# fskovbo/OptimalControlMPS

Measured on NVIDIA B200. Metric: cost+gradient evals/s (BH N=20 chi=100), higher is better.
Workload: dtype complex128 (f64)

## Files before the change

optimalcontrolmps_b200/csrc/decomp.cu:

```cuda
#include <cstdio>
#include <cstdlib>
#include "ocmps_internal.h"

__device__ unsigned long long g_jac_dbg[8];
__device__ double g_jac_flops[2];

namespace {

constexpr int JAC_THREADS = 512;
constexpr int JAC_EPL = 8;
constexpr int JAC_NV_SMEM = 512;
constexpr int JAC_MAX_SWEEPS = 60;
constexpr int JAC_BLOCKED_ROWS = 64;
constexpr double JAC_TOL2 = 1e-28;
constexpr double DEFLATE_REL = 1e-30;
constexpr int NV_MAX = 2048;
constexpr int BJ_C = 8;
constexpr int BJ_TPP = 4;
constexpr int BJ_MAX_ROWS = 256;
constexpr int BJ_SLOTS = BJ_MAX_ROWS / 2;
constexpr int BJ_THREADS = BJ_SLOTS * BJ_TPP;
constexpr int BJ_MAX_EPL = 8;
constexpr int BJ_MIN_CAP = 112;

__host__ __device__ __forceinline__ int gc_ldy(int len) { int l = (len + 3) & ~3; if ((l & 7) == 0) l += 4; return l; }
__host__ __device__ __forceinline__ int gc_ldg(int nvp) { return nvp | 1; }
__device__ __forceinline__ void gc_dmma(double& d0, double& d1, double a, double b) {
  asm volatile("mma.sync.aligned.m8n8k4.row.col.f64.f64.f64.f64 {%0,%1}, {%2}, {%3}, {%0,%1};\n" : "+d"(d0), "+d"(d1) : "d"(a), "d"(b));
// ... 249 lines not shown
      rb[e].x = __shfl_xor_sync(0xffffffffu, rb[e].x, 16);
      rb[e].y = __shfl_xor_sync(0xffffffffu, rb[e].y, 16);
    }
    nbn = __shfl_xor_sync(0xffffffffu, nbn, 16);
    rowB = __shfl_xor_sync(0xffffffffu, rowB, 16);
    jac_rotate<EPL>(ra, rb, na, nbn, rowA >= 0 && rowB >= 0, thr, hl, s_rot, s_big);
    int NP = -1, NQ = -1;
    if (R + 1 < nbp - 1) {
      blocks_of(R + 1, NP, NQ);
      if ((NP >= 0 && NP == hbB) || (NQ >= 0 && NQ == hbA)) { const int t = NP; NP = NQ; NQ = t; }
    }
    if (hbA != NP) store_row(ra, na, rowA);
    if (hbB != NQ) store_row(rb, nbn, rowB);
    P = NP; Q = NQ;
    __syncthreads();
  }
}

struct QrState {
  cplx* Y;
  int nv, len;
  double rtol_abs;
  double *ncur, *nnext, *nrmref, *rdr, *rdi;
  short *perm, *pcur, *pnext;
  unsigned long long (*s_cand)[32];
};

template <int EPL, int E0>
__device__ __forceinline__ bool qr_step_cached(const QrState& q, int j) {
  constexpr unsigned long long KEY_POS = 2047ull;
  constexpr int nwarps = JAC_THREADS / 32;
  const int tid = threadIdx.x, lane = tid & 31, warp = tid >> 5, half = lane >> 4, hl = lane & 15;
  const int len = q.len, nv = q.nv;
  int bpos;
  {
    const unsigned long long kk = q.s_cand[j & 1][lane];
    const unsigned khi = (unsigned)(kk >> 32);
    const unsigned mhi = __reduce_max_sync(0xffffffffu, khi);
    const unsigned mlo = __reduce_max_sync(0xffffffffu, khi == mhi ? (unsigned)kk : 0u);
    bpos = (int)(KEY_POS - (unsigned long long)(mlo & 2047u));
  }
  const int pv = q.pcur[bpos];
  const int pj = q.pcur[j];
  const cplx* x = q.Y + pv * len;
  const cplx alpha = x[j];
  cplx xv[EPL];
  double sq0 = 0.0, sq1 = 0.0;
#pragma unroll
  for (int e = E0; e < EPL; ++e) {
    const int c = hl + 16 * e;
    const bool in = (e > E0 || c >= j) && (e < EPL - 1 || c < len);
    xv[e] = x[in ? c : j];
    if (!in) xv[e] = make_double2(0.0, 0.0);
    const double q2 = xv[e].x * xv[e].x + xv[e].y * xv[e].y;
    if ((e - E0) & 1) sq1 += q2; else sq0 += q2;
  }
  const double best = half_sum(sq0 + sq1);
  if (!(best > q.rtol_abs)) return false;
  const double inx = rsqrt(best), normx = best * inx;
  const double a2 = alpha.x * alpha.x + alpha.y * alpha.y;
  const double ia = a2 > 0.0 ? rsqrt(a2) : 0.0, aabs = a2 * ia;
  const double phr = a2 > 0.0 ? alpha.x * ia : 1.0, phi = a2 > 0.0 ? alpha.y * ia : 0.0;
  const double dr = phr * normx, di = phi * normx;
  const double v0r = alpha.x + dr, v0i = alpha.y + di;
  const double rb = rsqrt(normx * (normx + aabs));
  const double beta = rb * rb;
  if (tid == 0) { q.rdr[j] = -dr; q.rdi[j] = -di; q.perm[j] = (short)pv; }
  unsigned long long cand = 0ull;
  for (int ib = j + 1 + 2 * warp; ib < nv; ib += 2 * nwarps) {
    const int i = ib + half;
    const bool act = i < nv;
    const int phys = act ? (i == bpos ? pj : (int)q.pcur[i]) : pv;
    cplx* y = q.Y + phys * len;
    const cplx yj = y[j];
    const double told = q.ncur[phys], tref = q.nrmref[phys];
    cplx yv[EPL];
    double w0r = 0.0, w0i = 0.0, w1r = 0.0, w1i = 0.0;
#pragma unroll
    for (int e = E0; e < EPL; ++e) {
      const int c = hl + 16 * e;
      if (e < EPL - 1) yv[e] = y[c];
      else { yv[e] = y[c < len ? c : j]; if (c >= len) yv[e] = make_double2(0.0, 0.0); }
      const double pr = xv[e].x * yv[e].x + xv[e].y * yv[e].y;
      const double pi = xv[e].x * yv[e].y - xv[e].y * yv[e].x;
      if ((e - E0) & 1) { w1r += pr; w1i += pi; } else { w0r += pr; w0i += pi; }
    }
    double wr = half_sum(w0r + w1r), wi = half_sum(w0i + w1i);
    wr += dr * yj.x + di * yj.y;
    wi += dr * yj.y - di * yj.x;
    const double fr = beta * wr, fi = beta * wi;
// ... 144 lines not shown
  }
  __syncthreads();
  if (tid == 0) {
    double t = 0.0;
    for (int v = 0; v < nv; ++v) t += nrm[v];
    s_F = t;
    s_keff = 0;
  }
  __syncthreads();
  const double F = s_F;
  const double rtol_abs = F * rank_tol;

  const long long t_qr0 = clock64();
  const int kmax = nv < len ? nv : len;
  int keff = 0;
  double* ncur = nrm;  double* nnext = nrm2;
  short* pcur = permA; short* pnext = permB;
  constexpr unsigned long long KEY_POS = 2047ull;
  const bool qr_cached = CACHED && len <= 16 * JAC_EPL;
  if (qr_cached) {
    QrState q;
    q.Y = Y; q.nv = nv; q.len = len; q.rtol_abs = rtol_abs;
    q.ncur = ncur; q.nnext = nnext; q.nrmref = nrmref; q.rdr = rdr; q.rdi = rdi;
    q.perm = perm; q.pcur = pcur; q.pnext = pnext; q.s_cand = s_cand;
    switch ((len + 15) >> 4) {
      case 1: keff = qr_pivoted_cached<1>(q); break;
      case 2: keff = qr_pivoted_cached<2>(q); break;
      case 3: keff = qr_pivoted_cached<3>(q); break;
      case 4: keff = qr_pivoted_cached<4>(q); break;
      case 5: keff = qr_pivoted_cached<5>(q); break;
      case 6: keff = qr_pivoted_cached<6>(q); break;
      case 7: keff = qr_pivoted_cached<7>(q); break;
      default: keff = qr_pivoted_cached<8>(q); break;
    }
    ncur = q.ncur; nnext = q.nnext; pcur = q.pcur; pnext = q.pnext;
  }
  if (tid < 3) s_key[tid] = 0ull;
  __syncthreads();
  for (int v = tid; v < nv; v += JAC_THREADS)
    atomicMax(&s_key[0], ((unsigned long long)__double_as_longlong(nrm[v]) & ~KEY_POS) | (KEY_POS - (unsigned long long)v));
  __syncthreads();
  for (int j = 0; j < (qr_cached ? 0 : kmax); ++j) {
    const int bpos = (int)(KEY_POS - (s_key[j % 3] & KEY_POS));
    if (tid == 0) s_key[(j + 2) % 3] = 0ull;
    const int pv = pcur[bpos];
    const int pj = pcur[j];
// ... 49 lines not shown
      if (act) {
        tnew = ncur[phys] - rji2;
        redo = !(tnew > 1.5e-8 * nrmref[phys]);
      }
      if (__any_sync(0xffffffffu, redo)) {
        double tail = 0.0;
        if (act && redo) for (int c = j + 1 + hl; c < len; c += 16) { const cplx yy = y[c]; tail += yy.x * yy.x + yy.y * yy.y; }
        tail = half_sum(tail);
        if (act && redo) { tnew = tail; if (hl == 0) nrmref[phys] = tail; }
      }
      if (act && hl == 0) {
        tnew = tnew > 0.0 ? tnew : 0.0;
        nnext[phys] = tnew; pnext[i] = (short)phys;
        atomicMax(knext, ((unsigned long long)__double_as_longlong(tnew) & ~KEY_POS) | (KEY_POS - (unsigned long long)i));
      }
    }
    }
    __syncthreads();
    { double* t = ncur; ncur = nnext; nnext = t; short* u = pcur; pcur = pnext; pnext = u; }
  }
  for (int i = keff + tid; i < nv; i += JAC_THREADS) perm[i] = pcur[i];
  __syncthreads();
  if (tid == 0) s_keff = keff;

  const int ldz = CACHED ? ldpad : nv;
  for (int e = tid; e < keff * ldz; e += JAC_THREADS) {
    const int c = e / ldz, i = e % ldz;
    cplx v = make_double2(0.0, 0.0);
    if (i == c) v = make_double2(rdr[c], rdi[c]);
    else if (i > c && i < nv) v = Y[(int)perm[i] * len + c];
    Yb[e] = v;
  }
  __syncthreads();
  {
    double* hF = b.scratch_d + 7 * NV_MAX;
    int* hK = reinterpret_cast<int*>(b.scratch_d + 7 * NV_MAX + OCMPS_MAX_BLK);
    int* hB = hK + OCMPS_MAX_BLK;
    int* hS = hB + OCMPS_MAX_BLK;
    const bool handover_small = CACHED && keff <= JAC_BLOCKED_ROWS;
    const bool handover_big = !handover_small && big_on && keff <= BJ_MAX_ROWS && nv <= BJ_MAX_ROWS;
    const bool handover = handover_small || handover_big;
    if (tid == 0) {
      hF[blockIdx.x] = F;
      hK[blockIdx.x] = handover_small ? keff : -1;
      hB[blockIdx.x] = handover_big ? keff : -1;
      hS[blockIdx.x] = ldz;
// ... 1219 lines not shown
  extern __shared__ __align__(16) unsigned char smem_raw[];
  __shared__ RcShared sh;
  const int blk = (int)blockIdx.x / RC_C;
  const unsigned rank = clus::cluster_rank();
  const int keff = rot_handover_rows(b, blk, smem_elems);
  if (keff < 0) return;
  if (keff < RC_MIN_ROWS) {
    if (rank == 0) jacobi_rot_block(a, b, blk, keff, smem_raw);
    return;
  }
  cplx* Zs = reinterpret_cast<cplx*>(smem_raw);
  switch ((b.dw->blk[blk].nv + 15) >> 4) {
    case 1: rc_run<1>(a, b, blk, keff, rank, Zs, sh); break;
    case 2: rc_run<2>(a, b, blk, keff, rank, Zs, sh); break;
    case 3: rc_run<3>(a, b, blk, keff, rank, Zs, sh); break;
    case 4: rc_run<4>(a, b, blk, keff, rank, Zs, sh); break;
    case 5: rc_run<5>(a, b, blk, keff, rank, Zs, sh); break;
    case 6: rc_run<6>(a, b, blk, keff, rank, Zs, sh); break;
    case 7: rc_run<7>(a, b, blk, keff, rank, Zs, sh); break;
    default: rc_run<8>(a, b, blk, keff, rank, Zs, sh); break;
  }
}

__global__ void __launch_bounds__(1024) truncate_kernel(DecompArgs a, DecompBuffers b, TruncParams tp) {
  __shared__ double cP[NV_MAX];
  __shared__ double sSorted[NV_MAX];
  __shared__ short cQ[NV_MAX], cI[NV_MAX], cI2[NV_MAX];
  __shared__ unsigned char sKeep[NV_MAX];
  __shared__ int sBlkOff[OCMPS_MAX_BLK + 1];
  __shared__ double sWarp[32];
  __shared__ int sWarpCnt[33];
  __shared__ double s_docut, s_kept;
  __shared__ int s_nfinal;
  DecompWork* w = b.dw;
  const int nv = w->nvtot;
  const int nblocks = w->nblocks;
  const int tid = threadIdx.x, lane = tid & 31, warp = tid >> 5;
  for (int i = tid; i < nblocks; i += blockDim.x) sBlkOff[i] = w->blk[i].p_off;
  if (tid == 0) { s_nfinal = 0; s_docut = 0.0; }
  const int i0 = 2 * tid, i1 = i0 + 1;
  const double p0 = i0 < nv ? b.P[i0] : 0.0, p1 = i1 < nv ? b.P[i1] : 0.0;
  const int f0 = p0 > 0.0, f1 = p1 > 0.0;
  int incl = f0 + f1;
#pragma unroll
  for (int o = 1; o < 32; o <<= 1) { const int up = __shfl_up_sync(0xffffffffu, incl, o); if (lane >= o) incl += up; }
  if (lane == 31) sWarpCnt[warp + 1] = incl;
// ... 152 lines not shown
      for (int i = 0; i < 32; ++i) t += sWarp[i];
      s_kept = t;
    }
    __syncthreads();
  }
  if (tid == 0) {
    int k = total;
    if (k == 0 && nv > 0) {
      k = 1;
      a.qNew[0] = b.vecq[0];
      inv_blk[0] = 0;
      inv_v[0] = 0;
    }
    if (k > tp.cap) { atomicOr(b.status, OCMPS_ST_CAPACITY); k = tp.cap; }
    w->newdim = k;
    *a.dimNew = k;
    const double kept = s_kept;
    double scale = 1.0;
    if (tp.normalize) {
      const double nrm = sqrt(kept);
      if (nrm > 1e-16) scale = 1.0 / nrm;
    }
    w->scale = scale;
    const int n = w->n, m = w->m;
    GemmDesc g1;
    g1.pad = 0;
    g1.A = g1.B = nullptr; g1.C = nullptr; g1.M = g1.N = g1.K = 0; g1.lda = g1.ldb = g1.ldc = 1; g1.opA = g1.opB = 0;
    if (a.kind == DK_ORTH_LEFT) {
      const int far = a.D * (*a.dimNb);
      g1.A = a.partner; g1.opA = 0; g1.lda = m;
      g1.B = a.nb_in; g1.opB = 0; g1.ldb = far;
      g1.C = a.nb_out; g1.ldc = far; g1.M = k; g1.N = far; g1.K = m;
    } else if (a.kind == DK_ORTH_RIGHT) {
      const int far = a.D * (*a.dimNb);
      g1.A = a.nb_in; g1.opA = 0; g1.lda = n;
      g1.B = a.partner; g1.opB = 0; g1.ldb = k;
      g1.C = a.nb_out; g1.ldc = k; g1.M = far; g1.N = k; g1.K = n;
    }
    b.descs[1] = g1;
  }
}

constexpr int BUILD_THREADS = 512;
__global__ void __launch_bounds__(BUILD_THREADS) build_factors_kernel(DecompArgs a, DecompBuffers b) {
  extern __shared__ __align__(16) unsigned char bsm[];
  __shared__ double red[BUILD_THREADS / 32];
  __shared__ double s_inv;
  const DecompWork* w = b.dw;
  const int k = w->newdim;
  const int kk = blockIdx.x;
  if (kk >= k) return;
  const int n = w->n, m = w->m, ld = w->ld, mode = w->mode;
  const int* comp_blk = b.comp_idx + NV_MAX;
  const int* comp_rank = b.comp_idx + 2 * NV_MAX;
  const int* vec_blk = b.vec_idx + NV_MAX;
  const int* vec_rank = b.vec_idx + 2 * NV_MAX;
  const int bi = b.pos[NV_MAX + kk], j = b.pos[2 * NV_MAX + kk];
  const DecompBlock B = w->blk[bi];
  const int nv = B.nv, len = B.len;
  const cplx* Zj = b.ywork + B.ws_off + (size_t)j * nv;
  const double sigma = sqrt(b.P[B.p_off + j]) * w->scale;
  cplx* zs = reinterpret_cast<cplx*>(bsm);
  cplx* out = zs + nv;
  int* vidx = reinterpret_cast<int*>(out + len);
  int* cidx = vidx + nv;
  const int tid = threadIdx.x, lane = tid & 31, wp = tid >> 5;
  constexpr int NW = BUILD_THREADS / 32;
  for (int v = tid; v < nv; v += BUILD_THREADS) { zs[v] = Zj[v]; vidx[v] = b.vec_idx[B.vec_off + v]; }
  for (int c = tid; c < len; c += BUILD_THREADS) cidx[c] = b.comp_idx[B.comp_off + c];
  __syncthreads();
  double part = 0.0;
  if (mode == 0) {
    for (int c = wp; c < len; c += NW) {
      const cplx* row = a.X + (size_t)cidx[c] * ld;
      double sr = 0.0, si = 0.0;
      for (int v0 = 0; v0 < nv; v0 += 128) {
        cplx x[4];
#pragma unroll
        for (int u = 0; u < 4; ++u) {
          const int v = v0 + lane + 32 * u;
          x[u] = make_double2(0.0, 0.0);
          if (v < nv) x[u] = row[vidx[v]];
        }
#pragma unroll
        for (int u = 0; u < 4; ++u) {
          const int v = v0 + lane + 32 * u;
          if (v < nv) {
            const cplx z = zs[v];
            sr += x[u].x * z.x + x[u].y * z.y;
            si += x[u].y * z.x - x[u].x * z.y;
          }
        }
      }
      sr = warp_sum(sr); si = warp_sum(si);
      if (lane == 0) { out[c] = make_double2(sr, si); part += sr * sr + si * si; }
// ... 4 lines not shown
      const int c = c0 + cl;
      const bool in = c < len;
      const cplx* colp = a.X + (in ? cidx[c] : 0);
      double sr = 0.0, si = 0.0;
      if (in) {
#pragma unroll 4
        for (int v = g; v < nv; v += 4) {
          const cplx x = colp[(size_t)vidx[v] * ld], z = zs[v];
          sr += x.x * z.x + x.y * z.y;
          si += x.y * z.x - x.x * z.y;
        }
      }
      sr += __shfl_xor_sync(0xffffffffu, sr, 8);  si += __shfl_xor_sync(0xffffffffu, si, 8);
      sr += __shfl_xor_sync(0xffffffffu, sr, 16); si += __shfl_xor_sync(0xffffffffu, si, 16);
      if (in && g == 0) { out[c] = make_double2(sr, si); part += sr * sr + si * si; }
    }
  }
  part = warp_sum(part);
  if ((tid & 31) == 0) red[tid >> 5] = part;
  __syncthreads();
  if (tid == 0) {
    double t = 0.0;
    for (int i = 0; i < BUILD_THREADS / 32; ++i) t += red[i];
    s_inv = t > 0.0 ? rsqrt(t) : 0.0;
  }
  __syncthreads();
  const double inv = s_inv;
  const int ncomp = mode == 0 ? n : m, nvec = mode == 0 ? m : n;
  for (int c = tid; c < ncomp; c += BUILD_THREADS) {
    cplx v = make_double2(0.0, 0.0);
    if (comp_blk[c] == bi) { const cplx o = out[comp_rank[c]]; v = make_double2(o.x * inv, o.y * inv); }
    if (mode == 0) a.iso[(size_t)c * k + kk] = v; else a.iso[(size_t)kk * m + c] = v;
  }
  if (a.qNb != nullptr && (a.kind == DK_ORTH_LEFT || a.kind == DK_ORTH_RIGHT)) {
    const int D = a.D, chiFar = *a.dimNb, qj = B.q;
    if (a.kind == DK_ORTH_LEFT) {
      const long long far = (long long)D * chiFar;
      for (int r = tid; r < chiFar; r += BUILD_THREADS) {
        const int sx = a.qNb[r] - qj;
        double ar = 0.0, ai = 0.0;
        if (sx >= 0 && sx < D) {
          const cplx* col = a.nb_in + (long long)sx * chiFar + r;
#pragma unroll 4
          for (int t = 0; t < nv; ++t) {
            const cplx z = zs[t], x = col[(long long)vidx[t] * far];
            ar += z.x * x.x - z.y * x.y;
            ai += z.x * x.y + z.y * x.x;
// ... 70 lines not shown
}

int grid_for(long long elems, int threads, int cap = 1184) {
  long long g = (elems + threads - 1) / threads;
  if (g < 1) g = 1;
  if (g > cap) g = cap;
  return (int)g;
}

}

static bool g_jac_attr_set[64] = {false};

void debug_jacobi_counters(unsigned long long* out, bool reset) {
  cudaMemcpyFromSymbol(out, g_jac_dbg, sizeof(unsigned long long) * 8);
  if (reset) { unsigned long long z[8] = {0}; cudaMemcpyToSymbol(g_jac_dbg, z, sizeof(z)); }
}

void debug_row_cluster_counters(unsigned long long* out, bool reset) {
  cudaMemcpyFromSymbol(out, g_rc_dbg, sizeof(unsigned long long) * 2);
  if (reset) { unsigned long long z[2] = {0, 0}; cudaMemcpyToSymbol(g_rc_dbg, z, sizeof(z)); }
}

__global__ void __launch_bounds__(256) spectrum_entropy_kernel(DecompBuffers b, double* out) {
  __shared__ double red[256];
  const int nv = b.dw->nvtot;
  double acc = 0.0;
  for (int i = threadIdx.x; i < nv; i += 256) {
    const double p = b.P[i];
    if (p > 1e-12) acc -= p * log(p);
  }
  red[threadIdx.x] = acc;
  __syncthreads();
  for (int o = 128; o > 0; o >>= 1) {
    if ((int)threadIdx.x < o) red[threadIdx.x] += red[threadIdx.x + o];
    __syncthreads();
  }
  if (threadIdx.x == 0) *out = red[0];
}

void launch_spectrum_entropy(const DecompBuffers& b, double* out, cudaStream_t s) {
  spectrum_entropy_kernel<<<1, 256, 0, s>>>(b, out);
}

void launch_decomp_setup(const DecompArgs& a, const DecompBuffers& b, cudaStream_t s) {
  decomp_setup_kernel<<<1, SETUP_THREADS, 0, s>>>(a, b);
// ... 38 lines not shown
    }
    e0 = g_prof_events[g_prof_used].first; e1 = g_prof_events[g_prof_used].second;
    ++g_prof_used;
    cudaEventRecord(e0, s);
  }
  struct Tail { cudaEvent_t e; cudaStream_t s; ~Tail() { if (e) cudaEventRecord(e, s); } } tail{e1, s};
  int dev = 0;
  cudaGetDevice(&dev);
  static std::mutex attr_mu;
  if (dev < 64) {
  std::lock_guard<std::mutex> attr_lock(attr_mu);
  if (!g_jac_attr_set[dev]) {
    cudaFuncSetAttribute(jacobi_blocks_kernel<true, true>, cudaFuncAttributeMaxDynamicSharedMemorySize, 200 * 1024);
    cudaFuncSetAttribute(jacobi_blocks_kernel<true, false>, cudaFuncAttributeMaxDynamicSharedMemorySize, 200 * 1024);
    cudaFuncSetAttribute(build_factors_kernel, cudaFuncAttributeMaxDynamicSharedMemorySize, 96 * 1024);
    cudaFuncSetAttribute(jacobi_rot_kernel, cudaFuncAttributeMaxDynamicSharedMemorySize, (int)(JAC_BLOCKED_ROWS * 16 * JAC_EPL * sizeof(cplx)));
    cudaFuncSetAttribute(jacobi_rows_cluster_kernel, cudaFuncAttributeMaxDynamicSharedMemorySize, (int)(JAC_BLOCKED_ROWS * 16 * JAC_EPL * sizeof(cplx)));
    cudaFuncSetAttribute(jacobi_big_kernel, cudaFuncAttributeMaxDynamicSharedMemorySize, (int)(BJ_MAX_ROWS * (BJ_TPP * BJ_MAX_EPL + 4) * sizeof(cplx)));
    cudaFuncSetAttribute(qr_big_kernel, cudaFuncAttributeMaxDynamicSharedMemorySize, (int)((32 * BJ_MAX_ROWS + BJ_MAX_ROWS) * sizeof(cplx)));
    g_jac_attr_set[dev] = true;
  }
  }
  static const bool big_env = [] { const char* e = getenv("OCMPS_BIG_CLUSTER"); return !(e && e[0] == '0'); }();
  int big_on = (big_env && max_rows >= BJ_MIN_CAP) ? 1 : 0;
  static const bool gram_env = [] { const char* e = getenv("OCMPS_GRAM"); return e && e[0] == '1'; }();
  if (gram_env && (a.kind == DK_GATE_LEFT || a.kind == DK_GATE_RIGHT)) big_on |= 2;
  static const bool fork_env = [] { const char* e = getenv("OCMPS_SVD_FORK"); return !(e && e[0] == '0'); }();
  const bool forked = fork_env && (big_on & 1) && fork && fork->stream;
  cudaStream_t sb = forked ? fork->stream : s;
  if (forked) { cudaEventRecord(fork->ev_fork, s); cudaStreamWaitEvent(sb, fork->ev_fork, 0); }
  jacobi_blocks_kernel<true, true><<<nblk_launch, JAC_THREADS, smem_limit, s>>>(a, b, (int)(smem_limit / sizeof(cplx)), rank_tol, big_on);
  if (forked) cudaEventRecord(fork->ev_first, s);
  if (long_rows) jacobi_blocks_kernel<true, false><<<nblk_launch, JAC_THREADS, smem_limit, s>>>(a, b, (int)(smem_limit / sizeof(cplx)), rank_tol, big_on);
  if (need_global) jacobi_blocks_kernel<false, false><<<nblk_launch, JAC_THREADS, 0, s>>>(a, b, (int)(smem_limit / sizeof(cplx)), rank_tol, big_on);
  if (big_on & 1) {
    cudaLaunchConfig_t cfg = {};
    cfg.gridDim = dim3(nblk_launch * BJ_C, 1, 1);
    cfg.blockDim = dim3(BJ_THREADS, 1, 1);
    cfg.dynamicSmemBytes = (size_t)(32 * BJ_MAX_ROWS + BJ_MAX_ROWS) * sizeof(cplx);
    cfg.stream = sb;
    cudaLaunchAttribute at[1];
    at[0].id = cudaLaunchAttributeClusterDimension;
    at[0].val.clusterDim.x = BJ_C; at[0].val.clusterDim.y = 1; at[0].val.clusterDim.z = 1;
    cfg.attrs = at; cfg.numAttrs = 1;
    cudaLaunchKernelEx(&cfg, qr_big_kernel, a, b, (int)(smem_limit / sizeof(cplx)), rank_tol);
  }
  if (spread_rows) {
    cudaLaunchConfig_t cfg = {};
    cfg.gridDim = dim3(nblk_launch * RC_C, 1, 1);
    cfg.blockDim = dim3(JAC_THREADS, 1, 1);
    cfg.dynamicSmemBytes = (size_t)JAC_BLOCKED_ROWS * 16 * JAC_EPL * sizeof(cplx);
    cfg.stream = s;
    cudaLaunchAttribute at[1];
    at[0].id = cudaLaunchAttributeClusterDimension;
    at[0].val.clusterDim.x = RC_C; at[0].val.clusterDim.y = 1; at[0].val.clusterDim.z = 1;
    cfg.attrs = at; cfg.numAttrs = 1;
    cudaLaunchKernelEx(&cfg, jacobi_rows_cluster_kernel, a, b, (int)(smem_limit / sizeof(cplx)));
  } else {
    jacobi_rot_kernel<<<nblk_launch, JAC_THREADS, JAC_BLOCKED_ROWS * 16 * JAC_EPL * sizeof(cplx), s>>>(a, b, (int)(smem_limit / sizeof(cplx)));
  }
  if (big_on & 1) {
    if (forked) cudaStreamWaitEvent(sb, fork->ev_first, 0);
    cudaLaunchConfig_t cfg = {};
    cfg.gridDim = dim3(nblk_launch * BJ_C, 1, 1);
    cfg.blockDim = dim3(BJ_THREADS, 1, 1);
    cfg.dynamicSmemBytes = (size_t)BJ_MAX_ROWS * (BJ_TPP * BJ_MAX_EPL + 4) * sizeof(cplx);
    cfg.stream = sb;
    cudaLaunchAttribute at[1];
    at[0].id = cudaLaunchAttributeClusterDimension;
    at[0].val.clusterDim.x = BJ_C; at[0].val.clusterDim.y = 1; at[0].val.clusterDim.z = 1;
    cfg.attrs = at; cfg.numAttrs = 1;
    cudaLaunchKernelEx(&cfg, jacobi_big_kernel, a, b);
    if (forked) { cudaEventRecord(fork->ev_join, sb); cudaStreamWaitEvent(s, fork->ev_join, 0); }
  }
}

void launch_truncate(const DecompArgs& a, const DecompBuffers& b, const TruncParams& tp, cudaStream_t s) {
  truncate_kernel<<<1, 1024, 0, s>>>(a, b, tp);
}

void launch_build_factors(const DecompArgs& a, const DecompBuffers& b, int cap_k, int cap_vec, int cap_comp, cudaStream_t s) {
  const size_t sm = (sizeof(cplx) + sizeof(int)) * (size_t)(cap_vec + cap_comp);
  build_factors_kernel<<<cap_k, BUILD_THREADS, sm, s>>>(a, b);
}

void launch_norm_only(const cplx* x, const int* dimL, const int* dimR, int D, double* partial, double* out, int max_elems,
                      cudaStream_t s) {
  (void)max_elems;
  norm_partial_site_kernel<<<NORM_CTAS, NORM_THREADS, 0, s>>>(x, dimL, dimR, D, partial);
  norm_finish_kernel<<<1, 32, 0, s>>>(partial, out);
}

void launch_normalize_site(cplx* x, const int* dimL, const int* dimR, int D, double* partial, int max_elems, cudaStream_t s) {
  norm_partial_site_kernel<<<NORM_CTAS, NORM_THREADS, 0, s>>>(x, dimL, dimR, D, partial);
  scale_site_kernel<<<grid_for(max_elems, 256), 256, 0, s>>>(x, dimL, dimR, D, partial);
}
```

optimalcontrolmps_b200/csrc/engine.cu:

```cuda
#include <cmath>
#include <complex>
#include <cstdio>
#include <cstring>
#include <cstdlib>
#include <algorithm>
#include <string>
#include <atomic>
#include <chrono>
#include <map>
#include <mutex>
#include <tuple>
#include <thread>
#include <vector>

#include "ocmps_internal.h"
#include "../../include/ocmps.h"

std::atomic<long long> g_ocmps_launches{0};

namespace {

thread_local std::string g_err;

int fail(int code, const std::string& msg) {
// ... 434 lines not shown
  ops.push_back({0, 1, 1, 0});
  ops.push_back({3, 1, 0, 0});
  return ops;
}

struct StepTrace {
  bool on = false;
  std::vector<std::pair<int, cudaEvent_t>> marks;
  void mark(int phase, cudaStream_t s) {
    if (!on) return;
    cudaEvent_t e = nullptr;
    cudaEventCreate(&e);
    cudaEventRecord(e, s);
    marks.push_back({phase, e});
  }
};
static StepTrace g_trace;
static bool step_trace_enabled() {
  static const bool v = [] { const char* e = getenv("OCMPS_STEP_TRACE"); return e && e[0] == '1'; }();
  return v;
}
enum { TR_START = 0, TR_MERGE, TR_SETUP, TR_SVD_GATE, TR_SVD_ORTH, TR_TRUNC, TR_BUILD, TR_OTHER, TR_NPHASE };

void run_decomp(Workspace* ws, const DecompArgs& a, const TruncParams& tp, int capV, int capC, int capK, cudaStream_t s,
                DecompBuffers* dbp = nullptr, bool setup_done = false, const DecompArgs* next = nullptr, DecompBuffers* db_next = nullptr) {
  DecompBuffers& db = dbp ? *dbp : ws->db;
  if (!setup_done) { launch_decomp_setup(a, db, s); g_trace.mark(TR_SETUP, s); }
  size_t need = (size_t)capV * capC * sizeof(cplx);
  need = std::max(need, (size_t)std::min(capV, capC) * (size_t)(((capV + 15) / 16) * 16) * sizeof(cplx));
  size_t smem = std::min(need, JAC_SMEM_LIMIT);
  if (smem < 1024) smem = 1024;
  int nblk = std::min(std::min(OCMPS_MAX_BLK, std::max(capV, capC) + a.D), ws->ctx->qmax.load() + a.D + 1);
  const bool need_global = need > JAC_SMEM_LIMIT;
  static const double rank_scale = [] { const char* e = getenv("OCMPS_RANK_TOL_SCALE"); return e ? atof(e) : 1e-6; }();
  double rank_tol = rank_scale * tp.cutoff;
  rank_tol = std::min(rank_scale * 1e-8, std::max(1e-30, rank_tol));
  const bool long_rows = capV > 128;
  const int max_rows = std::min(capV, capC);
  launch_jacobi_blocks(a, db, nblk, smem, need_global, long_rows, rank_tol, max_rows, capV, capC, ws->spread_jacobi, s, &ws->fork);
  g_trace.mark((a.kind == DK_GATE_LEFT || a.kind == DK_GATE_RIGHT) ? TR_SVD_GATE : TR_SVD_ORTH, s);
  launch_truncate(a, db, tp, s);
  g_trace.mark(TR_TRUNC, s);
  if (next) {
    cudaEventRecord(ws->ev_trunc, s);
    cudaStreamWaitEvent(ws->side, ws->ev_trunc, 0);
    launch_decomp_setup(*next, *db_next, ws->side);
    cudaEventRecord(ws->ev_setup, ws->side);
  }
  launch_build_factors(a, db, capK, capV, capC, s);
  g_trace.mark(TR_BUILD, s);
  g_ocmps_launches += 5 + (need_global ? 1 : 0) + (long_rows ? 1 : 0);
}

void phases_of(int D, double U, double tstep, double* re, double* im, bool imag = false) {
  for (int n = 0; n < D; ++n) {
    if (imag) {
      re[n] = std::exp(-0.25 * U * tstep * (double)n * (double)(n - 1));
      im[n] = 0.0;
      continue;
    }
    const double ang = -0.25 * U * tstep * (double)n * (double)(n - 1);
    re[n] = std::cos(ang);
    im[n] = std::sin(ang);
  }
}

static bool fused_push_enabled() {
  static const bool v = [] { const char* e = getenv("OCMPS_FUSED_PUSH"); return !(e && e[0] == '0'); }();
  return v;
}

void run_step_body(ocmps_stepper* st, ocmps_mps* m, Workspace* ws, cudaStream_t s, int op_begin = 0, int op_end = 1 << 30) {
  const int D = st->D;
  const Layout& lay = m->lay;
  const StepParams* sp = ws->d_params;
  TruncParams tpg{st->cutoff, st->maxm, 1, st->rel_cutoff, 0, 1};
  TruncParams tpo{MIN_CUT, MAX_M, 1, 0, 0, 0};

  auto setup_args = [&](const Op& op) {
    DecompArgs a;
    a.D = D;
    if (op.kind == 1) {
      const int bl = op.a - 1, br = op.a + 1;
      a.kind = op.c == 0 ? DK_GATE_LEFT : DK_GATE_RIGHT;
      a.dimL = m->dim(bl); a.dimR = m->dim(br); a.qL = m->q(bl); a.qR = m->q(br);
    } else {
      const int b = op.a;
      a.kind = op.b == 0 ? DK_ORTH_LEFT : DK_ORTH_RIGHT;
      const int lo = op.b == 0 ? b - 1 : b;
      a.dimL = m->dim(lo); a.dimR = m->dim(lo + 1); a.qL = m->q(lo); a.qR = m->q(lo + 1);
    }
// ... 43 lines not shown
      DecompArgs a;
      a.kind = op.c == 0 ? DK_GATE_LEFT : DK_GATE_RIGHT;
      a.D = D;
      a.dimL = m->dim(bl); a.dimR = m->dim(br); a.qL = m->q(bl); a.qR = m->q(br);
      a.dimNew = m->dim(bm); a.qNew = m->q(bm);
      a.X = ws->theta;
      a.iso = op.c == 0 ? m->other(j1) : m->other(j2);
      a.partner = op.c == 0 ? m->other(j2) : m->other(j1);
      a.nb_in = nullptr; a.nb_out = nullptr; a.dimNb = nullptr; a.qNb = nullptr;
      tpg.cap = lay.capb[bm];
      const int n_cap = lay.capb[bl] * D, m_cap = D * lay.capb[br];
      const int capV = op.c == 0 ? lay.capb[br] : lay.capb[bl];
      const int capC = op.c == 0 ? lay.capb[bl] : lay.capb[br];
      (void)n_cap; (void)m_cap;
      pipelined_decomp(oi, a, tpg, capV, capC, lay.capb[bm]);
      m->cur[j1] ^= 1; m->cur[j2] ^= 1;
      g_ocmps_launches += 3;
    } else if (op.kind == 2) {
      const int b = op.a;
      DecompArgs a;
      a.D = D;
      a.dimNew = m->dim(b); a.qNew = m->q(b);
      a.partner = ws->cbuf;
      tpo.cap = lay.capb[b];
      if (op.b == 0) {
        const int j = b - 1, jn = b;
        a.kind = DK_ORTH_LEFT;
        a.dimL = m->dim(b - 1); a.dimR = m->dim(b); a.qL = m->q(b - 1); a.qR = m->q(b);
        a.X = m->site(j); a.iso = m->other(j);
        a.nb_in = m->site(jn); a.nb_out = m->other(jn); a.dimNb = m->dim(b + 1);
        a.qNb = fused_push ? m->q(b + 1) : nullptr;
        DecompBuffers* dbc = pipelined_decomp(oi, a, tpo, lay.capb[b], lay.capb[b - 1], lay.capb[b]);
        if (!fused_push) launch_zgemm(dbc->descs + 1, 1, lay.capb[b], D * lay.capb[b + 1], s);
        m->cur[j] ^= 1; m->cur[jn] ^= 1;
      } else {
        const int j = b, jn = b - 1;
        a.kind = DK_ORTH_RIGHT;
        a.dimL = m->dim(b); a.dimR = m->dim(b + 1); a.qL = m->q(b); a.qR = m->q(b + 1);
        a.X = m->site(j); a.iso = m->other(j);
        a.nb_in = m->site(jn); a.nb_out = m->other(jn); a.dimNb = m->dim(b - 1);
        a.qNb = fused_push ? m->q(b - 1) : nullptr;
        DecompBuffers* dbc = pipelined_decomp(oi, a, tpo, lay.capb[b], lay.capb[b + 1], lay.capb[b]);
        if (!fused_push) launch_zgemm(dbc->descs + 1, 1, lay.capb[b - 1] * D, lay.capb[b], s);
        m->cur[j] ^= 1; m->cur[jn] ^= 1;
      }
      g_ocmps_launches += fused_push ? 0 : 1;
// ... 579 lines not shown
static int check_shapes(ocmps_stepper* st, const Layout& lay, const char* what) {
  if (lay.L != st->L || lay.D != st->D || lay.cap != st->cap)
    return fail(OCMPS_ERR_INVALID, std::string(what) + ": MPS/store shape (L, D, chi_cap) differs from the stepper's");
  return OCMPS_OK;
}

int ocmps_step(ocmps_stepper* st, ocmps_mps* psi, double from, double to, int forward) {
  if (!st || !psi) return fail(OCMPS_ERR_INVALID, "null argument");
  int rc = check_shapes(st, psi->lay, "step");
  if (rc) return rc;
  if (psi->llim != 0 || psi->rlim != 2) return fail(OCMPS_ERR_INVALID, "step: orthogonality centre must be at site 1");
  CK(cudaSetDevice(st->ctx->dev));
  WsLease lease;
  rc = lease.acquire(st->ctx, st->L, st->D, st->cap, 1);
  if (rc) return rc;
  Workspace* ws = lease[0];
  rc = step_enqueue(st, psi, ws, from, to, forward != 0, nullptr, 0, ws->stream);
  if (rc) { cudaStreamSynchronize(ws->stream); return rc; }
  return lease.finish();
}

int ocmps_debug_jacobi(unsigned long long* out, int reset) { cudaDeviceSynchronize(); debug_jacobi_counters(out, reset != 0); return 0; }
int ocmps_debug_row_cluster(unsigned long long* out2, int reset) { cudaDeviceSynchronize(); debug_row_cluster_counters(out2, reset != 0); return 0; }

int ocmps_debug_run_ops(ocmps_stepper* st, ocmps_mps* psi, double from, double to, int forward, int op_begin, int op_end) {
  CK(cudaSetDevice(st->ctx->dev));
  WsLease lease;
  int rc = lease.acquire(st->ctx, st->L, st->D, st->cap, 1);
  if (rc) return rc;
  Workspace* ws = lease[0];
  { StepParams hp; fill_step_params(st, from, to, forward != 0, nullptr, 0, hp); launch_set_step_params(hp, ws->d_params, ws->stream); }
  run_step_body(st, psi, ws, ws->stream, op_begin, op_end);
  return lease.finish();
}

int ocmps_apply_K(ocmps_stepper* st, ocmps_mps* in, ocmps_mps* out) {
  if (!st || !in || !out) return fail(OCMPS_ERR_INVALID, "null argument");
  int rc = check_shapes(st, in->lay, "apply_K");
  if (rc) return rc;
  rc = check_shapes(st, out->lay, "apply_K");
  if (rc) return rc;
  CK(cudaSetDevice(st->ctx->dev));
  WsLease lease;
  rc = lease.acquire(st->ctx, st->L, st->D, st->cap, 1);
  if (rc) return rc;
  Workspace* ws = lease[0];
// ... 973 lines not shown
```

optimalcontrolmps_b200/csrc/ocmps_internal.h:

```cpp
#pragma once
#include <cuda_runtime.h>
#include <stdint.h>
#include <stddef.h>

typedef double2 cplx;

#define OCMPS_MAX_L 64
#define OCMPS_MAX_D 8
#define OCMPS_MAX_Q 256
#define OCMPS_MAX_BLK 128

#define OCMPS_ST_CAPACITY   1
#define OCMPS_ST_NOCONV     2
#define OCMPS_ST_CHARGE     4
#define OCMPS_ST_TOOMANYBLK 8

struct GemmDesc {
  const cplx* A; const cplx* B; cplx* C;
  int M, N, K;
  int lda, ldb, ldc;
  int opA, opB;
  int pad;
};

// ... 20 lines not shown
  int maxm, minm;
  int rel_cutoff;
  int cap;
  int normalize;
};

struct StepParams {
  double u1r[OCMPS_MAX_D], u1i[OCMPS_MAX_D];
  double u2r[OCMPS_MAX_D], u2i[OCMPS_MAX_D];
  const cplx* G;
  cplx* slot_data; int* slot_dims; int* slot_q;
};

struct SitePtrs { cplx* p[OCMPS_MAX_L]; };
struct SiteOffs { long long o[OCMPS_MAX_L + 1]; };

struct Phases { double re[4][OCMPS_MAX_D]; double im[4][OCMPS_MAX_D]; };

#include <atomic>
extern std::atomic<long long> g_ocmps_launches;

void debug_jacobi_counters(unsigned long long* out, bool reset);
void debug_row_cluster_counters(unsigned long long* out, bool reset);
void profile_enable(bool on);
bool profile_is_on();
void profile_read(double* out);

void launch_zgemm(const GemmDesc* d_descs, int batch, int maxM, int maxN, cudaStream_t s);

enum DecompKind { DK_GATE_LEFT = 0, DK_GATE_RIGHT = 1, DK_ORTH_LEFT = 2, DK_ORTH_RIGHT = 3 };

struct DecompArgs {
  int kind;
  int D;
  const int* dimL;
  const int* dimR;
  const int* qL;
  const int* qR;
  int* dimNew;
  int* qNew;
  const cplx* X;
  cplx* iso;
  cplx* partner;
  const cplx* nb_in;
  cplx* nb_out;
  const int* dimNb;
  const int* qNb;
};

struct DecompBuffers {
  DecompWork* dw;
  int* vec_idx; int* comp_idx;
  int* vecq;
  double* P;
  int* pos;
  cplx* ywork;
  long long ywork_half;
  double* scratch_d;
  GemmDesc* descs;
  double* partial;
  int* status;
};

void launch_decomp_setup(const DecompArgs& a, const DecompBuffers& b, cudaStream_t s);
struct SvdFork { cudaStream_t stream = nullptr; cudaEvent_t ev_fork = nullptr, ev_first = nullptr, ev_join = nullptr; };
void launch_jacobi_blocks(const DecompArgs& a, const DecompBuffers& b, int nblk_launch, size_t smem_limit, bool need_global,
                          bool long_rows, double rank_tol, int max_rows, int capV, int capC, bool spread_rows, cudaStream_t s,
                          const SvdFork* fork = nullptr);
void launch_spectrum_entropy(const DecompBuffers& b, double* out, cudaStream_t s);
void launch_truncate(const DecompArgs& a, const DecompBuffers& b, const TruncParams& tp, cudaStream_t s);
// ... 77 lines not shown
```

Before: 0.9257.

## Use pivoted Householder QR instead of Jacobi SVD for orthogonalization gauge moves

For orthogonalization decompositions with small blocks, the Jacobi SVD pipeline is replaced by the existing pivoted QR stage. The Householder reflectors and R factor are written out, bond dimensions are taken from the numerical rank instead of singular-value truncation, and Q columns are built by applying the reflectors in build_factors. This skips the Jacobi sweeps, the singular-value sort and truncation, and several launches for gauge-only moves. In exchange it adds a serial single-warp reflector application per output column, and bond dimensions may differ from the SVD path because only rank truncation is applied. It is enabled by default through an environment flag.

```diff
diff --git a/optimalcontrolmps_b200/csrc/decomp.cu b/optimalcontrolmps_b200/csrc/decomp.cu
--- a/optimalcontrolmps_b200/csrc/decomp.cu
+++ b/optimalcontrolmps_b200/csrc/decomp.cu
@@ -4,6 +4,7 @@
 
 __device__ unsigned long long g_jac_dbg[8];
 __device__ double g_jac_flops[2];
+__device__ unsigned long long g_qrg_dbg[1];
 
 namespace {
 
@@ -299,6 +300,7 @@
   int nv, len;
   double rtol_abs;
   double *ncur, *nnext, *nrmref, *rdr, *rdi;
+  double* beta;
   short *perm, *pcur, *pnext;
   unsigned long long (*s_cand)[32];
 };
@@ -342,7 +344,10 @@
   const double v0r = alpha.x + dr, v0i = alpha.y + di;
   const double rb = rsqrt(normx * (normx + aabs));
   const double beta = rb * rb;
-  if (tid == 0) { q.rdr[j] = -dr; q.rdi[j] = -di; q.perm[j] = (short)pv; }
+  if (tid == 0) {
+    q.rdr[j] = -dr; q.rdi[j] = -di; q.perm[j] = (short)pv;
+    if (q.beta) q.beta[j] = beta;
+  }
   unsigned long long cand = 0ull;
   for (int ib = j + 1 + 2 * warp; ib < nv; ib += 2 * nwarps) {
     const int i = ib + half;
@@ -533,6 +538,7 @@
     QrState q;
     q.Y = Y; q.nv = nv; q.len = len; q.rtol_abs = rtol_abs;
     q.ncur = ncur; q.nnext = nnext; q.nrmref = nrmref; q.rdr = rdr; q.rdi = rdi;
+    q.beta = a.qr_gauge ? b.P + B.p_off : nullptr;
     q.perm = perm; q.pcur = pcur; q.pnext = pnext; q.s_cand = s_cand;
     switch ((len + 15) >> 4) {
       case 1: keff = qr_pivoted_cached<1>(q); break;
@@ -628,6 +634,33 @@
   for (int i = keff + tid; i < nv; i += JAC_THREADS) perm[i] = pcur[i];
   __syncthreads();
   if (tid == 0) s_keff = keff;
+  if constexpr (SMEM && CACHED) {
+    if (a.qr_gauge) {
+      const int kq = keff > 0 ? keff : 1;
+      for (int e = tid; e < kq * len; e += JAC_THREADS) {
+        const int j = e / len, c = e - j * len;
+        cplx v = make_double2(0.0, 0.0);
+        if (j < keff && c >= j) {
+          v = Y[(int)perm[j] * len + c];
+          if (c == j) { v.x -= rdr[j]; v.y -= rdi[j]; }
+        }
+        Ya[e] = v;
+      }
+      for (int e = tid; e < kq * nv; e += JAC_THREADS) {
+        const int j = e / nv, i = e - j * nv;
+        cplx v = make_double2(0.0, 0.0);
+        if (j < keff && i == j) v = make_double2(rdr[j], rdi[j]);
+        else if (j < keff && i > j) v = Y[(int)perm[i] * len + j];
+        Yb[j * nv + (int)perm[i]] = v;
+      }
+      if (tid == 0) {
+        if (keff == 0) b.P[B.p_off] = 0.0;
+        reinterpret_cast<int*>(b.scratch_d + 7 * NV_MAX + OCMPS_MAX_BLK)[blockIdx.x] = keff;
+        atomicAdd(&g_qrg_dbg[0], 1ull);
+      }
+      return;
+    }
+  }
 
   const int ldz = CACHED ? ldpad : nv;
   for (int e = tid; e < keff * ldz; e += JAC_THREADS) {
@@ -1893,6 +1926,25 @@
   }
 }
 
+__device__ GemmDesc carry_push_desc(const DecompArgs& a, const DecompWork* w, int k) {
+  const int n = w->n, m = w->m;
+  GemmDesc g1;
+  g1.pad = 0;
+  g1.A = g1.B = nullptr; g1.C = nullptr; g1.M = g1.N = g1.K = 0; g1.lda = g1.ldb = g1.ldc = 1; g1.opA = g1.opB = 0;
+  if (a.kind == DK_ORTH_LEFT) {
+    const int far = a.D * (*a.dimNb);
+    g1.A = a.partner; g1.opA = 0; g1.lda = m;
+    g1.B = a.nb_in; g1.opB = 0; g1.ldb = far;
+    g1.C = a.nb_out; g1.ldc = far; g1.M = k; g1.N = far; g1.K = m;
+  } else if (a.kind == DK_ORTH_RIGHT) {
+    const int far = a.D * (*a.dimNb);
+    g1.A = a.nb_in; g1.opA = 0; g1.lda = n;
+    g1.B = a.partner; g1.opB = 0; g1.ldb = k;
+    g1.C = a.nb_out; g1.ldc = k; g1.M = far; g1.N = k; g1.K = n;
+  }
+  return g1;
+}
+
 __global__ void __launch_bounds__(1024) truncate_kernel(DecompArgs a, DecompBuffers b, TruncParams tp) {
   __shared__ double cP[NV_MAX];
   __shared__ double sSorted[NV_MAX];
@@ -2091,30 +2143,56 @@
       if (nrm > 1e-16) scale = 1.0 / nrm;
     }
     w->scale = scale;
-    const int n = w->n, m = w->m;
-    GemmDesc g1;
-    g1.pad = 0;
-    g1.A = g1.B = nullptr; g1.C = nullptr; g1.M = g1.N = g1.K = 0; g1.lda = g1.ldb = g1.ldc = 1; g1.opA = g1.opB = 0;
-    if (a.kind == DK_ORTH_LEFT) {
-      const int far = a.D * (*a.dimNb);
-      g1.A = a.partner; g1.opA = 0; g1.lda = m;
-      g1.B = a.nb_in; g1.opB = 0; g1.ldb = far;
-      g1.C = a.nb_out; g1.ldc = far; g1.M = k; g1.N = far; g1.K = m;
-    } else if (a.kind == DK_ORTH_RIGHT) {
-      const int far = a.D * (*a.dimNb);
-      g1.A = a.nb_in; g1.opA = 0; g1.lda = n;
-      g1.B = a.partner; g1.opB = 0; g1.ldb = k;
-      g1.C = a.nb_out; g1.ldc = k; g1.M = far; g1.N = k; g1.K = n;
-    }
-    b.descs[1] = g1;
+    b.descs[1] = carry_push_desc(a, w, k);
+  }
+}
+
+__global__ void __launch_bounds__(256) qr_gauge_bonds_kernel(DecompArgs a, DecompBuffers b, TruncParams tp) {
+  __shared__ int s_off[OCMPS_MAX_BLK + 1];
+  DecompWork* w = b.dw;
+  const int nblocks = w->nblocks;
+  const int* keffs = reinterpret_cast<const int*>(b.scratch_d + 7 * NV_MAX + OCMPS_MAX_BLK);
+  const int tid = threadIdx.x, lane = tid & 31, warp = tid >> 5;
+  if (tid == 0) {
+    int t = 0;
+    for (int bi = 0; bi < nblocks; ++bi) { s_off[bi] = t; t += keffs[bi]; }
+    s_off[nblocks] = t;
+  }
+  __syncthreads();
+  int* inv_blk = b.pos + NV_MAX;
+  int* inv_v = b.pos + 2 * NV_MAX;
+  for (int bi = warp; bi < nblocks; bi += 256 / 32) {
+    const int q = w->blk[bi].q, o = s_off[bi], kb = s_off[bi + 1] - o;
+    for (int j = lane; j < kb && o + j < tp.cap; j += 32) {
+      a.qNew[o + j] = q;
+      inv_blk[o + j] = bi;
+      inv_v[o + j] = j;
+    }
+  }
+  if (tid == 0) {
+    int k = s_off[nblocks];
+    if (k == 0 && nblocks > 0) {
+      k = 1;
+      a.qNew[0] = w->blk[0].q;
+      inv_blk[0] = 0;
+      inv_v[0] = 0;
+    }
+    if (k > tp.cap) { atomicOr(b.status, OCMPS_ST_CAPACITY); k = tp.cap; }
+    w->newdim = k;
+    *a.dimNew = k;
+    w->scale = 1.0;
+    b.descs[1] = carry_push_desc(a, w, k);
   }
 }
 
 constexpr int BUILD_THREADS = 512;
+constexpr int QG_STAGE = 4096;
+constexpr int QG_MAX_LEN = 128;
 __global__ void __launch_bounds__(BUILD_THREADS) build_factors_kernel(DecompArgs a, DecompBuffers b) {
   extern __shared__ __align__(16) unsigned char bsm[];
   __shared__ double red[BUILD_THREADS / 32];
   __shared__ double s_inv;
+  __shared__ double s_beta[QG_MAX_LEN];
   const DecompWork* w = b.dw;
   const int k = w->newdim;
   const int kk = blockIdx.x;
@@ -2127,9 +2205,11 @@
   const int bi = b.pos[NV_MAX + kk], j = b.pos[2 * NV_MAX + kk];
   const DecompBlock B = w->blk[bi];
   const int nv = B.nv, len = B.len;
-  const cplx* Zj = b.ywork + B.ws_off + (size_t)j * nv;
-  const double sigma = sqrt(b.P[B.p_off + j]) * w->scale;
-  cplx* zs = reinterpret_cast<cplx*>(bsm);
+  const bool qr = a.qr_gauge != 0;
+  const cplx* Zj = b.ywork + (qr ? b.ywork_half : 0) + B.ws_off + (size_t)j * nv;
+  const double sigma = (qr ? 1.0 : sqrt(b.P[B.p_off + j])) * w->scale;
+  cplx* stage = reinterpret_cast<cplx*>(bsm);
+  cplx* zs = stage + (qr ? QG_STAGE : 0);
   cplx* out = zs + nv;
   int* vidx = reinterpret_cast<int*>(out + len);
   int* cidx = vidx + nv;
@@ -2137,9 +2217,47 @@
   constexpr int NW = BUILD_THREADS / 32;
   for (int v = tid; v < nv; v += BUILD_THREADS) { zs[v] = Zj[v]; vidx[v] = b.vec_idx[B.vec_off + v]; }
   for (int c = tid; c < len; c += BUILD_THREADS) cidx[c] = b.comp_idx[B.comp_off + c];
+  if (qr) for (int m2 = tid; m2 <= j; m2 += BUILD_THREADS) s_beta[m2] = b.P[B.p_off + m2];
   __syncthreads();
   double part = 0.0;
-  if (mode == 0) {
+  if (qr) {
+    const cplx* V = b.ywork + B.ws_off;
+    cplx y[QG_MAX_LEN / 32];
+#pragma unroll
+    for (int e = 0; e < QG_MAX_LEN / 32; ++e) y[e] = make_double2(lane + 32 * e == j ? 1.0 : 0.0, 0.0);
+    const int per = QG_STAGE / len;
+    for (int m1 = j; m1 >= 0; m1 -= per) {
+      const int m0 = m1 - per + 1 > 0 ? m1 - per + 1 : 0;
+      for (int e = tid; e < (m1 - m0 + 1) * len; e += BUILD_THREADS) stage[e] = V[(size_t)m0 * len + e];
+      __syncthreads();
+      if (wp == 0) {
+        for (int m2 = m1; m2 >= m0; --m2) {
+          const cplx* v = stage + (m2 - m0) * len;
+          cplx vv[QG_MAX_LEN / 32];
+          double wr = 0.0, wi = 0.0;
+#pragma unroll
+          for (int e = 0; e < QG_MAX_LEN / 32; ++e) {
+            const int c = lane + 32 * e;
+            vv[e] = c < len ? v[c] : make_double2(0.0, 0.0);
+            wr += vv[e].x * y[e].x + vv[e].y * y[e].y;
+            wi += vv[e].x * y[e].y - vv[e].y * y[e].x;
+          }
+          wr = warp_sum(wr); wi = warp_sum(wi);
+          const double fr = s_beta[m2] * wr, fi = s_beta[m2] * wi;
+#pragma unroll
+          for (int e = 0; e < QG_MAX_LEN / 32; ++e) {
+            y[e].x -= fr * vv[e].x - fi * vv[e].y;
+            y[e].y -= fr * vv[e].y + fi * vv[e].x;
+          }
+        }
+      }
+      __syncthreads();
+    }
+    if (wp == 0) {
+#pragma unroll
+      for (int e = 0; e < QG_MAX_LEN / 32; ++e) if (lane + 32 * e < len) out[lane + 32 * e] = y[e];
+    }
+  } else if (mode == 0) {
     for (int c = wp; c < len; c += NW) {
       const cplx* row = a.X + (size_t)cidx[c] * ld;
       double sr = 0.0, si = 0.0;
@@ -2190,7 +2308,7 @@
   if (tid == 0) {
     double t = 0.0;
     for (int i = 0; i < BUILD_THREADS / 32; ++i) t += red[i];
-    s_inv = t > 0.0 ? rsqrt(t) : 0.0;
+    s_inv = qr ? 1.0 : (t > 0.0 ? rsqrt(t) : 0.0);
   }
   __syncthreads();
   const double inv = s_inv;
@@ -2307,6 +2425,11 @@
   if (reset) { unsigned long long z[2] = {0, 0}; cudaMemcpyToSymbol(g_rc_dbg, z, sizeof(z)); }
 }
 
+void debug_qr_gauge_counters(unsigned long long* out, bool reset) {
+  cudaMemcpyFromSymbol(out, g_qrg_dbg, sizeof(unsigned long long));
+  if (reset) { unsigned long long z = 0; cudaMemcpyToSymbol(g_qrg_dbg, &z, sizeof(z)); }
+}
+
 __global__ void __launch_bounds__(256) spectrum_entropy_kernel(DecompBuffers b, double* out) {
   __shared__ double red[256];
   const int nv = b.dw->nvtot;
@@ -2391,7 +2514,7 @@
   }
   }
   static const bool big_env = [] { const char* e = getenv("OCMPS_BIG_CLUSTER"); return !(e && e[0] == '0'); }();
-  int big_on = (big_env && max_rows >= BJ_MIN_CAP) ? 1 : 0;
+  int big_on = (big_env && max_rows >= BJ_MIN_CAP && !a.qr_gauge) ? 1 : 0;
   static const bool gram_env = [] { const char* e = getenv("OCMPS_GRAM"); return e && e[0] == '1'; }();
   if (gram_env && (a.kind == DK_GATE_LEFT || a.kind == DK_GATE_RIGHT)) big_on |= 2;
   static const bool fork_env = [] { const char* e = getenv("OCMPS_SVD_FORK"); return !(e && e[0] == '0'); }();
@@ -2400,6 +2523,7 @@
   if (forked) { cudaEventRecord(fork->ev_fork, s); cudaStreamWaitEvent(sb, fork->ev_fork, 0); }
   jacobi_blocks_kernel<true, true><<<nblk_launch, JAC_THREADS, smem_limit, s>>>(a, b, (int)(smem_limit / sizeof(cplx)), rank_tol, big_on);
   if (forked) cudaEventRecord(fork->ev_first, s);
+  if (a.qr_gauge) return;
   if (long_rows) jacobi_blocks_kernel<true, false><<<nblk_launch, JAC_THREADS, smem_limit, s>>>(a, b, (int)(smem_limit / sizeof(cplx)), rank_tol, big_on);
   if (need_global) jacobi_blocks_kernel<false, false><<<nblk_launch, JAC_THREADS, 0, s>>>(a, b, (int)(smem_limit / sizeof(cplx)), rank_tol, big_on);
   if (big_on & 1) {
@@ -2445,11 +2569,12 @@
 }
 
 void launch_truncate(const DecompArgs& a, const DecompBuffers& b, const TruncParams& tp, cudaStream_t s) {
-  truncate_kernel<<<1, 1024, 0, s>>>(a, b, tp);
+  if (a.qr_gauge) qr_gauge_bonds_kernel<<<1, 256, 0, s>>>(a, b, tp);
+  else truncate_kernel<<<1, 1024, 0, s>>>(a, b, tp);
 }
 
 void launch_build_factors(const DecompArgs& a, const DecompBuffers& b, int cap_k, int cap_vec, int cap_comp, cudaStream_t s) {
-  const size_t sm = (sizeof(cplx) + sizeof(int)) * (size_t)(cap_vec + cap_comp);
+  const size_t sm = (sizeof(cplx) + sizeof(int)) * (size_t)(cap_vec + cap_comp) + (a.qr_gauge ? QG_STAGE * sizeof(cplx) : 0);
   build_factors_kernel<<<cap_k, BUILD_THREADS, sm, s>>>(a, b);
 }
 
diff --git a/optimalcontrolmps_b200/csrc/engine.cu b/optimalcontrolmps_b200/csrc/engine.cu
--- a/optimalcontrolmps_b200/csrc/engine.cu
+++ b/optimalcontrolmps_b200/csrc/engine.cu
@@ -480,9 +480,10 @@
 }
 enum { TR_START = 0, TR_MERGE, TR_SETUP, TR_SVD_GATE, TR_SVD_ORTH, TR_TRUNC, TR_BUILD, TR_OTHER, TR_NPHASE };
 
-void run_decomp(Workspace* ws, const DecompArgs& a, const TruncParams& tp, int capV, int capC, int capK, cudaStream_t s,
+void run_decomp(Workspace* ws, const DecompArgs& a_in, const TruncParams& tp, int capV, int capC, int capK, cudaStream_t s,
                 DecompBuffers* dbp = nullptr, bool setup_done = false, const DecompArgs* next = nullptr, DecompBuffers* db_next = nullptr) {
   DecompBuffers& db = dbp ? *dbp : ws->db;
+  DecompArgs a = a_in;
   if (!setup_done) { launch_decomp_setup(a, db, s); g_trace.mark(TR_SETUP, s); }
   size_t need = (size_t)capV * capC * sizeof(cplx);
   need = std::max(need, (size_t)std::min(capV, capC) * (size_t)(((capV + 15) / 16) * 16) * sizeof(cplx));
@@ -495,6 +496,7 @@
   rank_tol = std::min(rank_scale * 1e-8, std::max(1e-30, rank_tol));
   const bool long_rows = capV > 128;
   const int max_rows = std::min(capV, capC);
+  a.qr_gauge = a_in.qr_gauge && capV <= 128 && capC <= 128 && !need_global;
   launch_jacobi_blocks(a, db, nblk, smem, need_global, long_rows, rank_tol, max_rows, capV, capC, ws->spread_jacobi, s, &ws->fork);
   g_trace.mark((a.kind == DK_GATE_LEFT || a.kind == DK_GATE_RIGHT) ? TR_SVD_GATE : TR_SVD_ORTH, s);
   launch_truncate(a, db, tp, s);
@@ -507,7 +509,7 @@
   }
   launch_build_factors(a, db, capK, capV, capC, s);
   g_trace.mark(TR_BUILD, s);
-  g_ocmps_launches += 5 + (need_global ? 1 : 0) + (long_rows ? 1 : 0);
+  g_ocmps_launches += a.qr_gauge ? 4 : 5 + (need_global ? 1 : 0) + (long_rows ? 1 : 0);
 }
 
 void phases_of(int D, double U, double tstep, double* re, double* im, bool imag = false) {
@@ -525,6 +527,11 @@
 
 static bool fused_push_enabled() {
   static const bool v = [] { const char* e = getenv("OCMPS_FUSED_PUSH"); return !(e && e[0] == '0'); }();
+  return v;
+}
+
+static bool qr_gauge_enabled() {
+  static const bool v = [] { const char* e = getenv("OCMPS_QR_GAUGE"); return !(e && e[0] == '0'); }();
   return v;
 }
 
@@ -614,6 +621,7 @@
       a.D = D;
       a.dimNew = m->dim(b); a.qNew = m->q(b);
       a.partner = ws->cbuf;
+      a.qr_gauge = qr_gauge_enabled() ? 1 : 0;
       tpo.cap = lay.capb[b];
       if (op.b == 0) {
         const int j = b - 1, jn = b;
@@ -1239,6 +1247,7 @@
 
 int ocmps_debug_jacobi(unsigned long long* out, int reset) { cudaDeviceSynchronize(); debug_jacobi_counters(out, reset != 0); return 0; }
 int ocmps_debug_row_cluster(unsigned long long* out2, int reset) { cudaDeviceSynchronize(); debug_row_cluster_counters(out2, reset != 0); return 0; }
+int ocmps_debug_qr_gauge(unsigned long long* out1, int reset) { cudaDeviceSynchronize(); debug_qr_gauge_counters(out1, reset != 0); return 0; }
 
 int ocmps_debug_run_ops(ocmps_stepper* st, ocmps_mps* psi, double from, double to, int forward, int op_begin, int op_end) {
   CK(cudaSetDevice(st->ctx->dev));
diff --git a/optimalcontrolmps_b200/csrc/ocmps_internal.h b/optimalcontrolmps_b200/csrc/ocmps_internal.h
--- a/optimalcontrolmps_b200/csrc/ocmps_internal.h
+++ b/optimalcontrolmps_b200/csrc/ocmps_internal.h
@@ -66,6 +66,7 @@
 
 void debug_jacobi_counters(unsigned long long* out, bool reset);
 void debug_row_cluster_counters(unsigned long long* out, bool reset);
+void debug_qr_gauge_counters(unsigned long long* out, bool reset);
 void profile_enable(bool on);
 bool profile_is_on();
 void profile_read(double* out);
@@ -90,6 +91,7 @@
   cplx* nb_out;
   const int* dimNb;
   const int* qNb;
+  int qr_gauge = 0;
 };
 
 struct DecompBuffers {
```

Measured after the change: 1.007, median of 6. +8.7%, better.
